# ChampiB/CBO_with_OOP

Measured on NVIDIA B200. Metric: EI grid-points/sec per trial (all exploration sets), higher is better.
Workload: dtype f64

## Files before the change

cbo_with_oop_b200/build.py:

```python
from __future__ import annotations

import os
import subprocess
import sys
from concurrent.futures import ThreadPoolExecutor

HERE = os.path.dirname(os.path.abspath(__file__))
CSRC = os.path.join(HERE, "csrc")
INCLUDE = os.path.join(HERE, "..", "include")
LIB = os.path.join(HERE, "libcbo_b200.so")
SOURCES = ["api.cu", "tables.cu", "prior_precompute.cu", "prior_eval.cu", "prior_pair.cu", "prior_rows.cu", "posterior_fit.cu", "sweep.cu", "obs_gp_fit.cu", "sem.cu", "refine.cu"]
HEADERS = ["cbo_common.cuh", "dmma_tile.cuh", "dmma_tma_tile.cuh", "prior_pair.cuh", os.path.join(INCLUDE, "cbo_b200.h")]
NVCC_FLAGS = ["-gencode", "arch=compute_100a,code=sm_100a", "-O3", "-lineinfo", "-std=c++17",
              "-Xcompiler", "-fPIC", "-Xcompiler", "-fvisibility=hidden"]


def _nvcc() -> str:
    for cand in (os.environ.get("NVCC"), "/usr/local/cuda/bin/nvcc", "nvcc"):
        if cand and (os.path.isabs(cand) and os.path.exists(cand) or not os.path.isabs(cand)):
            return cand
    raise RuntimeError("nvcc not found")


def _stale() -> bool:
    if not os.path.exists(LIB):
        return True
    t = os.path.getmtime(LIB)
    deps = [os.path.join(CSRC, s) for s in SOURCES] + [h if os.path.isabs(h) else os.path.join(CSRC, h) for h in HEADERS]
    deps.append(os.path.abspath(__file__))
    return any(os.path.getmtime(d) > t for d in deps)


def build_library(force: bool = False, verbose: bool = False) -> str:
    if not force and not _stale():
        return LIB
    nvcc = _nvcc()
    objdir = os.path.join(HERE, "build")
    os.makedirs(objdir, exist_ok=True)
    extra = ["-Xptxas", "-v"] if verbose else []
    extra += os.environ.get("CBO_NVCC_EXTRA", "").split()

    def compile_one(src: str) -> str:
        obj = os.path.join(objdir, src.replace(".cu", ".o"))
        cmd = [nvcc, *NVCC_FLAGS, *extra, "-I", INCLUDE, "-c", os.path.join(CSRC, src), "-o", obj]
        r = subprocess.run(cmd, capture_output=True, text=True)
        if r.returncode != 0:
            raise RuntimeError(f"nvcc failed on {src}:\n{r.stdout}\n{r.stderr}")
        if verbose:
            sys.stderr.write(r.stderr)
        return obj

    with ThreadPoolExecutor(max_workers=len(SOURCES)) as ex:
        objs = list(ex.map(compile_one, SOURCES))
    cmd = [nvcc, "-shared", "-o", LIB, *objs, "-gencode", "arch=compute_100a,code=sm_100a"]
    r = subprocess.run(cmd, capture_output=True, text=True)
    if r.returncode != 0:
        raise RuntimeError(f"link failed:\n{r.stdout}\n{r.stderr}")
    return LIB


if __name__ == "__main__":
    print(build_library(force="--force" in sys.argv, verbose="--verbose" in sys.argv))
```

cbo_with_oop_b200/csrc/prior_eval.cu:

```cuda
#include "dmma_tile.cuh"
#include "prior_pair.cuh"

namespace cbo {

constexpr int kPriorWsHeader = 256;

constexpr int kPartialDoubles = 2 * CBO_PRIOR_TILE;
constexpr int kKbPerJ = kMBlkRows / kBK;
constexpr int kPartialFloor = 1024;

struct PriorSplit { int chunk, nsplit, skip_pair; };
__host__ __device__ inline long long prior_tiles(const cbo_set_desc& S, PriorSplit sp) {
    if (!computes_prior(S) || (sp.skip_pair && pair_eligible(S))) return 0;
    return (S.g_count + CBO_PRIOR_TILE - 1) / CBO_PRIOR_TILE;
}
__host__ __device__ inline int prior_nJ(const cbo_set_desc& S) { return (S.n_obs + kMBlkRows - 1) / kMBlkRows; }

__host__ __device__ inline long long prior_G(int n, int chunk) {
    if (n <= 0) return 0;
    const long long q = n / chunk, r = n - q * chunk;
    return (long long)chunk * q * (q + 1) / 2 + r * (q + 1);
}
__host__ __device__ inline long long prior_F(int jb, int chunk) { return prior_G(jb - 1, chunk) + jb; }
__host__ __device__ inline int prior_nsplit(const cbo_set_desc& S, int nsplit) {
    const int nJ = prior_nJ(S), cap = nJ / 2 > 1 ? nJ / 2 : 1;
    return nsplit < cap ? nsplit : cap;
}
__host__ __device__ inline long long prior_items_per_tile(const cbo_set_desc& S, PriorSplit sp) {
    return sp.chunk > 0 ? prior_F(prior_nJ(S), sp.chunk) : prior_nsplit(S, sp.nsplit);
}
__host__ __device__ inline long long prior_items(const cbo_set_desc& S, PriorSplit sp) {
    return prior_tiles(S, sp) * prior_items_per_tile(S, sp);
}

template <int WM_, int WN_, int MA_, int NB_, int STAGES_>
struct PriorCfg {
    static constexpr int WM = WM_, WN = WN_, MA = MA_, NB = NB_, STAGES = STAGES_;
    static constexpr int BM = WM * MA * 8;
    static constexpr int BN = WN * NB * 8;
    static constexpr int NCONS = WM * WN * 32;
    static constexpr int NT = NCONS + 128;
    static constexpr int A_TILE = BM * kBK;
    static constexpr int B_TILE = BN * kBK;
    static constexpr unsigned STAGE_BYTES = (A_TILE + B_TILE) * sizeof(double);
    static constexpr size_t SMEM = (size_t)STAGES * STAGE_BYTES + 2 * WN * BM * sizeof(double) +
                                   (CBO_MAX_D + 1) * BM * sizeof(int32_t) + 2 * STAGES * sizeof(uint64_t) + 16;
    static constexpr int LAUNCH_REGS = (65536 / NT) / 8 * 8;
    static constexpr int PROD_REGS = 40, CONS_REGS = 232;
    static_assert(BM == CBO_PRIOR_TILE, "host item count assumes CBO_PRIOR_TILE points per work item");
    static_assert(BN == kMBlkRows, "the J block must match the row block of M's blocked layout");
    static_assert(NCONS % 128 == 0, "setmaxnreg works on whole warpgroups");
    static_assert(128 * PROD_REGS + NCONS * CONS_REGS <= NT * LAUNCH_REGS, "setmaxnreg budget exceeds the CTA's register pool");
};

struct PriorItem {
    const cbo_set_desc* S;
    int tile, nJ, jb0, jb1, kt0, kt1, sp, ns;
    int kmax;
    bool split;
    bool partial;
    __device__ __forceinline__ bool mine(int jb) const { const int r = jb % (2 * ns); return r == sp || r == 2 * ns - 1 - sp; }
    template <bool SPLIT> __device__ __forceinline__ int kbeg(int jb) const { return SPLIT ? kt0 : 0; }
    template <bool SPLIT> __device__ __forceinline__ int kend(int jb) const {
        const int e = SPLIT ? kt1 : (jb + 1) * kKbPerJ;
        return e < kmax ? e : kmax;
    }
};

constexpr int kMaxBases = 32;
struct PriorBases { int n; int base[kMaxBases + 1]; };

__device__ __forceinline__ PriorItem decode_prior_item(const cbo_set_desc* __restrict__ sets, int num_sets, PriorSplit split,
                                                       const PriorBases& pb, int item) {
    const int chunk = split.chunk;
    int local = item, s = 0;
    if (pb.n == num_sets) {
#pragma unroll 1
        for (; s < num_sets - 1; ++s)
            if (item < pb.base[s + 1]) break;
        local = item - pb.base[s];
    } else {
        for (; s < num_sets - 1; ++s) {
            const int cnt = (int)prior_items(sets[s], split);
            if (local < cnt) break;
            local -= cnt;
        }
    }
    PriorItem it;
    it.S = sets + s;
    it.nJ = prior_nJ(sets[s]);
    it.kmax = (sets[s].n_obs + kBK - 1) / kBK;
    it.split = chunk > 0;
    it.sp = 0, it.ns = 1;
    if (!it.split) {
        it.ns = prior_nsplit(sets[s], split.nsplit);
        it.tile = local / it.ns, it.sp = local % it.ns;
        it.jb0 = 0, it.jb1 = it.nJ, it.kt0 = it.kt1 = 0;
        it.partial = it.ns > 1;
        return it;
    }
    it.partial = prior_F(it.nJ, chunk) > 1;
    const int per_tile = (int)prior_F(it.nJ, chunk);
    it.tile = local / per_tile;
    const int seg = local - it.tile * per_tile;
    int lo = 0, hi = it.nJ - 1;
    while (lo < hi) {
        const int mid = (lo + hi + 1) >> 1;
        if (prior_F(mid, chunk) <= seg) lo = mid; else hi = mid - 1;
    }
    const int jb = lo, piece = seg - (int)prior_F(jb, chunk), lower = (jb + chunk - 1) / chunk;
    it.jb0 = jb, it.jb1 = jb + 1;
    if (piece < lower) {
        const int b1 = (piece + 1) * chunk < jb ? (piece + 1) * chunk : jb;
        it.kt0 = piece * chunk * kKbPerJ, it.kt1 = b1 * kKbPerJ;
    } else {
        it.kt0 = jb * kKbPerJ, it.kt1 = (jb + 1) * kKbPerJ;
    }
    return it;
}

__device__ __forceinline__ void bar_all(int nthreads) { asm volatile("bar.sync 0, %0;" ::"r"(nthreads) : "memory"); }
__device__ __forceinline__ void bar_consumers(int nthreads) { asm volatile("bar.sync 1, %0;" ::"r"(nthreads) : "memory"); }

template <class Cfg, int MW, int NW, int MA2, int NB2>
__device__ __forceinline__ void consume_ragged_block(const PriorItem& it, const double* __restrict__ sA, const double* __restrict__ sB,
                                                     double* __restrict__ sRed, uint64_t* full, uint64_t* empty, int& stage,
                                                     unsigned& phase, const double* __restrict__ scratch, const double* __restrict__ w,
                                                     int warp, int lane) {
    constexpr int BM = Cfg::BM, BN = Cfg::BN, WN = Cfg::WN, STAGES = Cfg::STAGES;
    static_assert(MW * NW * 32 == Cfg::NCONS && MW * MA2 * 8 == BM && NW <= WN, "re-tiling must cover the 128 rows with all consumer warps");
    const int jb = it.nJ - 1, noff = jb * kKbPerJ, ke = it.kmax;
    const int row0 = (warp / NW) * MA2 * 8, wn2 = warp % NW, col0 = wn2 * NB2 * 8;
    double acc[MA2][NB2][2];
#pragma unroll
    for (int mi = 0; mi < MA2; ++mi)
#pragma unroll
        for (int ni = 0; ni < NB2; ++ni) acc[mi][ni][0] = acc[mi][ni][1] = 0.0;
    auto run = [&](int k0, int k1) {
#pragma unroll 1
        for (int kt = k0; kt < k1; ++kt) {
            mbar_wait(&full[stage], phase);
            mma_stage<BM, BN, MA2, NB2, MA2>(sA + stage * Cfg::A_TILE, sB + stage * Cfg::B_TILE, acc, row0, col0, lane);
            __syncwarp();
            if (lane == 0) mbar_arrive(&empty[stage]);
            if (++stage == STAGES) { stage = 0; phase ^= 1u; }
        }
    };
    run(0, noff);
#pragma unroll
    for (int mi = 0; mi < MA2; ++mi)
#pragma unroll
        for (int ni = 0; ni < NB2; ++ni) { acc[mi][ni][0] *= 2.0; acc[mi][ni][1] *= 2.0; }
    run(noff, ke);
    bar_consumers(Cfg::NCONS);
#pragma unroll
    for (int mi = 0; mi < MA2; ++mi) {
        const int r = row0 + mi * 8 + (lane >> 2);
        double q = 0.0, mm = 0.0;
#pragma unroll
        for (int ni = 0; ni < NB2; ++ni) {
            const int j = jb * BN + col0 + ni * 8 + (lane & 3) * 2;
            const double2 u = __ldcg(reinterpret_cast<const double2*>(scratch + (size_t)(j >> 4) * Cfg::A_TILE + frag_off(BM, (j & 15) >> 2, r, j & 3)));
            const double2 ww = ldg_nc_d2(w + j);
            q = fma(acc[mi][ni][0], u.x, q);
            q = fma(acc[mi][ni][1], u.y, q);
            mm = fma(u.x, ww.x, mm);
            mm = fma(u.y, ww.y, mm);
        }
        q += __shfl_xor_sync(0xffffffffu, q, 1);
        q += __shfl_xor_sync(0xffffffffu, q, 2);
        mm += __shfl_xor_sync(0xffffffffu, mm, 1);
        mm += __shfl_xor_sync(0xffffffffu, mm, 2);
        if ((lane & 3) == 0) {
            sRed[wn2 * BM + r] += q;
            sRed[(WN + wn2) * BM + r] += mm;
        }
    }
}

template <class Cfg, int LIVE, bool SPLIT>
__device__ __forceinline__ void consume_item(const PriorItem& it, const double* __restrict__ sA, const double* __restrict__ sB,
                                             double* __restrict__ sRed, uint64_t* full, uint64_t* empty, int& stage, unsigned& phase,
                                             const double* __restrict__ scratch, const double* __restrict__ w, int warp, int lane,
                                             int ragged_cols) {
    constexpr int BM = Cfg::BM, BN = Cfg::BN, MA = Cfg::MA, NB = Cfg::NB, WN = Cfg::WN, STAGES = Cfg::STAGES;
    static_assert(BN / kBK == kKbPerJ, "J block width");
    const int wm = warp / WN, wn = warp % WN;
    const int row0 = wm * MA * 8, col0 = wn * NB * 8;
    if constexpr (LIVE == 0) {
#pragma unroll 1
        for (int jb = it.jb0; jb < it.jb1; ++jb) {
            if (!it.mine(jb)) continue;
#pragma unroll 1
            for (int kt = it.template kbeg<SPLIT>(jb); kt < it.template kend<SPLIT>(jb); ++kt) {
                mbar_wait(&full[stage], phase);
                __syncwarp();
                if (lane == 0) mbar_arrive(&empty[stage]);
                if (++stage == STAGES) { stage = 0; phase ^= 1u; }
            }
        }
        return;
    }
    constexpr int LV = LIVE > 0 ? LIVE : 1;
    double acc[MA][NB][2];
#pragma unroll
    for (int mi = 0; mi < MA; ++mi)
#pragma unroll
        for (int ni = 0; ni < NB; ++ni) acc[mi][ni][0] = acc[mi][ni][1] = 0.0;

    const int jend = (!SPLIT && LIVE == MA && ragged_cols > 0) ? it.nJ - 1 : it.jb1;
#pragma unroll 1
    for (int jb = it.jb0; jb < jend; ++jb) {
        if (!it.mine(jb)) continue;
        const int kb = it.template kbeg<SPLIT>(jb), ke = it.template kend<SPLIT>(jb), noff = jb * kKbPerJ;
        auto double_acc = [&]() {
#pragma unroll
            for (int mi = 0; mi < LV; ++mi)
#pragma unroll
                for (int ni = 0; ni < NB; ++ni) { acc[mi][ni][0] *= 2.0; acc[mi][ni][1] *= 2.0; }
        };
        auto run = [&](int k0, int k1) {
#pragma unroll 1
            for (int kt = k0; kt < k1; ++kt) {
                mbar_wait(&full[stage], phase);
                mma_stage<BM, BN, MA, NB, LV>(sA + stage * Cfg::A_TILE, sB + stage * Cfg::B_TILE, acc, row0, col0, lane);
                __syncwarp();
                if (lane == 0) mbar_arrive(&empty[stage]);
                if (++stage == STAGES) { stage = 0; phase ^= 1u; }
            }
        };
        if constexpr (SPLIT) {
            run(kb, ke);
        } else {
            run(kb, noff);
            double_acc();
            run(noff, ke);
        }
        if (ke <= noff) double_acc();
        const bool with_m = ke > noff;
        const int ubase = !SPLIT ? 0 : (ke <= noff ? noff - (ke - kb) : kb);
#pragma unroll
        for (int mi = 0; mi < LV; ++mi) {
            const int r = row0 + mi * 8 + (lane >> 2);
            double q = 0.0, mm = 0.0;
#pragma unroll
            for (int ni = 0; ni < NB; ++ni) {
                const int j = jb * BN + col0 + ni * 8 + (lane & 3) * 2;
                const double2 u = __ldcg(reinterpret_cast<const double2*>(
                    scratch + (size_t)((j >> 4) - ubase) * Cfg::A_TILE + frag_off(BM, (j & 15) >> 2, r, j & 3)));
                const double2 ww = ldg_nc_d2(w + j);
                q = fma(acc[mi][ni][0], u.x, q);
                q = fma(acc[mi][ni][1], u.y, q);
                mm = fma(u.x, ww.x, mm);
                mm = fma(u.y, ww.y, mm);
                acc[mi][ni][0] = acc[mi][ni][1] = 0.0;
            }
            q += __shfl_xor_sync(0xffffffffu, q, 1);
            q += __shfl_xor_sync(0xffffffffu, q, 2);
            mm += __shfl_xor_sync(0xffffffffu, mm, 1);
            mm += __shfl_xor_sync(0xffffffffu, mm, 2);
            if ((lane & 3) == 0) {
                sRed[wn * BM + r] += q;
                if (with_m) sRed[(WN + wn) * BM + r] += mm;
            }
        }
    }
    if constexpr (!SPLIT && LIVE == MA) {
        if (ragged_cols > 32) consume_ragged_block<Cfg, 4, 2, 4, 4>(it, sA, sB, sRed, full, empty, stage, phase, scratch, w, warp, lane);
        else if (ragged_cols > 16) consume_ragged_block<Cfg, 8, 1, 2, 4>(it, sA, sB, sRed, full, empty, stage, phase, scratch, w, warp, lane);
        else if (ragged_cols > 0) consume_ragged_block<Cfg, 8, 1, 2, 2>(it, sA, sB, sRed, full, empty, stage, phase, scratch, w, warp, lane);
    }
}

template <class Cfg, bool SPLIT>
__global__ void __launch_bounds__(Cfg::NT, 1)
prior_eval_kernel(const cbo_set_desc* __restrict__ sets, int num_sets, PriorSplit split, const PriorBases pb, int total_items,
                  int* __restrict__ counter, double* __restrict__ partials, double* __restrict__ scratch_base, size_t slot_doubles) {
    constexpr int BM = Cfg::BM, BN = Cfg::BN, WN = Cfg::WN, NT = Cfg::NT, NCONS = Cfg::NCONS;
    constexpr int STAGES = Cfg::STAGES;
    extern __shared__ __align__(16) unsigned char smem_raw[];
    double* sA = reinterpret_cast<double*>(smem_raw);
    double* sB = sA + STAGES * Cfg::A_TILE;
    double* sRed = sB + STAGES * Cfg::B_TILE;
    uint64_t* bars = reinterpret_cast<uint64_t*>(sRed + 2 * WN * BM);
    int32_t* sRow = reinterpret_cast<int32_t*>(bars + 2 * STAGES);
    volatile int32_t* sItem = sRow + (CBO_MAX_D + 1) * BM;
    uint64_t* full = bars;
    uint64_t* empty = bars + STAGES;

    const int tid = threadIdx.x, lane = tid & 31, warp = tid >> 5;
    double* __restrict__ scratch = scratch_base + (size_t)blockIdx.x * slot_doubles;

    if (tid == 0) {
        for (int i = 0; i < STAGES; ++i) {
            mbar_init(&full[i], 1);
            mbar_init(&empty[i], Cfg::WM * WN);
        }
        mbar_fence_init();
        *sItem = atomicAdd(counter, 1);
    }
    __syncthreads();
    int stage = 0;
    unsigned phase = 0;

    if (warp >= NCONS / 32) {
        setmaxnreg_dec<Cfg::PROD_REGS>();
        for (;;) {
            const int item = *sItem;
            if (item >= total_items) break;
            const PriorItem it = decode_prior_item(sets, num_sets, split, pb, item);
            const double* __restrict__ M = it.S->M;
            const int Npad = it.S->n_obs_pad;
            bar_all(NT);
            if (warp == NCONS / 32 && lane == 0) {
#pragma unroll 1
                for (int jb = it.jb0; jb < it.jb1; ++jb) {
                    if (!it.mine(jb)) continue;
                    const int kb = it.template kbeg<SPLIT>(jb), ke = it.template kend<SPLIT>(jb);
#pragma unroll 1
                    for (int kt = kb; kt < ke; ++kt) {
                        mbar_wait(&empty[stage], phase ^ 1u);
                        mbar_arrive_expect_tx(&full[stage], Cfg::STAGE_BYTES);
                        bulk_g2s(sB + stage * Cfg::B_TILE, M + mblk_base(jb, kt, Npad), Cfg::B_TILE * sizeof(double), &full[stage]);
                        bulk_g2s(sA + stage * Cfg::A_TILE, scratch + (size_t)(kt - kb) * Cfg::A_TILE, Cfg::A_TILE * sizeof(double), &full[stage]);
                        if (++stage == STAGES) { stage = 0; phase ^= 1u; }
                    }
                }
            }
            __syncwarp();
            bar_all(NT);
        }
    } else {
        setmaxnreg_inc<Cfg::CONS_REGS>();
        for (;;) {
            const int item = *sItem;
            if (item >= total_items) break;
            const PriorItem it = decode_prior_item(sets, num_sets, split, pb, item);
            const cbo_set_desc& S = *it.S;
            const int d = S.points ? 1 : S.d;
            const long long gbeg = S.g_begin, gcnt = S.g_count;
            const int Npad = S.n_obs_pad;
            const int nk_item = SPLIT ? it.kt1 - it.kt0 : it.nJ * kKbPerJ;
            const bool extra = SPLIT && it.kt1 <= it.jb0 * kKbPerJ;
            const int nKT = nk_item + (extra ? kKbPerJ : 0);
            const long long left = gcnt - (long long)it.tile * BM;
            const int nlive = left < BM ? (int)left : BM;

            const bool small_grid = S.g_total < 0x7fffffffLL;
            for (int r = tid; r < BM; r += NCONS) {
                const bool live = r < nlive;
                const long long g0 = gbeg + (live ? (long long)it.tile * BM + r : 0);
                if (small_grid) {
                    unsigned gg = (unsigned)g0;
#pragma unroll
                    for (int k = CBO_MAX_D - 1; k >= 0; --k) {
                        if (k < d) {
                            const unsigned pk = S.points ? (unsigned)S.g_total : (unsigned)S.p[k], q = gg / pk;
                            sRow[k * BM + r] = (int)(gg - q * pk) * Npad;
                            gg = q;
                        }
                    }
                } else {
                    long long gg = g0;
#pragma unroll
                    for (int k = CBO_MAX_D - 1; k >= 0; --k) {
                        if (k < d) {
                            const long long pk = S.points ? S.g_total : (long long)S.p[k];
                            sRow[k * BM + r] = (int)(gg % pk) * Npad;
                            gg /= pk;
                        }
                    }
                }
                sRow[CBO_MAX_D * BM + r] = live ? 1 : 0;
            }
            for (int i = tid; i < 2 * WN * BM; i += NCONS) sRed[i] = 0.0;
            bar_consumers(NCONS);

            {
                const double* tab[CBO_MAX_D];
#pragma unroll
                for (int k = 0; k < CBO_MAX_D; ++k) tab[k] = S.tab[k < d ? k : 0];
                const int per_slab = ((nlive + 3) >> 2) * 32;
                constexpr int UW = (BM / 4 * 32 + NCONS - 1) / NCONS;
                int roff[UW][CBO_MAX_D], dst0[UW], j0[UW];
                bool valid[UW], live[UW];
#pragma unroll
                for (int x = 0; x < UW; ++x) {
                    const int wi = tid + x * NCONS, l = wi & 31;
                    const int kb = l >> 3, half = l & 1, row = (wi >> 5) * 4 + ((l & 7) >> 1);
                    valid[x] = wi < per_slab;
                    live[x] = valid[x] && sRow[CBO_MAX_D * BM + row] != 0;
                    j0[x] = kb * 4 + half * 2;
                    dst0[x] = frag_off(BM, kb, row, half * 2);
#pragma unroll
                    for (int k = 0; k < CBO_MAX_D; ++k) roff[x][k] = (k < d && valid[x]) ? sRow[k * BM + row] : 0;
                }
#pragma unroll 1
                for (int ks = 0; ks < nKT; ++ks) {
                    const int kt = !SPLIT ? ks : (ks < nk_item ? it.kt0 + ks : it.jb0 * kKbPerJ + (ks - nk_item));
                    double2 v[UW];
#pragma unroll
                    for (int x = 0; x < UW; ++x) {
                        v[x] = make_double2(0.0, 0.0);
                        if (live[x]) {
                            const int j = kt * kBK + j0[x];
                            v[x] = ldg_nc_d2(tab[0] + roff[x][0] + j);
#pragma unroll
                            for (int k = 1; k < CBO_MAX_D; ++k) {
                                if (k < d) {
                                    const double2 t = ldg_nc_d2(tab[k] + roff[x][k] + j);
                                    v[x].x *= t.x; v[x].y *= t.y;
                                }
                            }
                        }
                    }
#pragma unroll
                    for (int x = 0; x < UW; ++x)
                        if (valid[x]) *reinterpret_cast<double2*>(scratch + (size_t)ks * Cfg::A_TILE + dst0[x]) = v[x];
                }
                fence_proxy_async();
            }
            bar_all(NT);

            {
                const int live_here = nlive - (warp / WN) * Cfg::MA * 8;
                const int need = live_here <= 0 ? 0 : (live_here + 7) >> 3;
                const int lc = S.n_obs - (it.nJ - 1) * BN;
                const int ragged_cols = (!SPLIT && nlive == BM && it.nJ > 1 && lc <= 64 && it.mine(it.nJ - 1)) ? lc : 0;
#define CBO_CONSUME(LIVE) consume_item<Cfg, LIVE, SPLIT>(it, sA, sB, sRed, full, empty, stage, phase, scratch, S.w, warp, lane, ragged_cols)
                if (need >= 7) CBO_CONSUME(8);
                else if (need == 6) CBO_CONSUME(6);
                else if (need == 5) CBO_CONSUME(5);
                else if (need == 4) CBO_CONSUME(4);
                else if (need == 3) CBO_CONSUME(3);
                else if (need == 2) CBO_CONSUME(2);
                else if (need == 1) CBO_CONSUME(1);
                else CBO_CONSUME(0);
#undef CBO_CONSUME
            }
            bar_consumers(NCONS);

            double* out_m = S.m;
            double* out_v = S.v;
            for (int r = tid; r < nlive; r += NCONS) {
                const long long loc = (long long)it.tile * BM + r;
                double qs = 0.0, ms = 0.0;
#pragma unroll
                for (int x = 0; x < WN; ++x) { qs += sRed[x * BM + r]; ms += sRed[(WN + x) * BM + r]; }
                if (it.partial) {
                    partials[(size_t)item * kPartialDoubles + r] = qs;
                    partials[(size_t)item * kPartialDoubles + BM + r] = ms;
                } else {
                    out_m[loc] = ms;
                    out_v[loc] = (S.s2 + S.noise) - qs;
                }
            }
            bar_consumers(NCONS);
            if (tid == 0) *sItem = atomicAdd(counter, 1);
            bar_all(NT);
        }
    }
}

__global__ void __launch_bounds__(CBO_PRIOR_TILE)
prior_finalize_kernel(const cbo_set_desc* __restrict__ sets, int num_sets, PriorSplit split,
                      const double* __restrict__ partials) {
    long long base = 0;
    for (int s = 0; s < num_sets; ++s) {
        const cbo_set_desc& S = sets[s];
        const int tiles = (int)prior_tiles(S, split);
        if (tiles == 0) continue;
        const int per = (int)prior_items_per_tile(S, split);
        if (per > 1) {
            const long long gcnt = S.g_count;
            double* out_m = S.m;
            double* out_v = S.v;
            for (int tile = blockIdx.x; tile < tiles; tile += gridDim.x) {
                const int r = threadIdx.x;
                const long long loc = (long long)tile * CBO_PRIOR_TILE + r;
                if (loc < gcnt) {
                    double qs = 0.0, ms = 0.0;
                    const double* p = partials + (size_t)(base + (long long)tile * per) * kPartialDoubles;
                    for (int i = 0; i < per; ++i, p += kPartialDoubles) {
                        qs += p[r];
                        ms += p[CBO_PRIOR_TILE + r];
                    }
                    out_m[loc] = ms;
                    out_v[loc] = (S.s2 + S.noise) - qs;
                }
            }
        }
        base += (long long)tiles * per;
    }
}

using PriorCfgA = PriorCfg<2, 4, 8, 4, 4>;

static size_t prior_slot_doubles(const cbo_set_desc* h_sets, int num_sets) {
    int npad = 0;
    for (int s = 0; s < num_sets; ++s)
        if (computes_prior(h_sets[s]) && h_sets[s].n_obs_pad > npad) npad = h_sets[s].n_obs_pad;
    return (size_t)CBO_PRIOR_TILE * npad;
}

static size_t prior_partial_items(long long ctas) { return (size_t)(4 * ctas + kPartialFloor); }

size_t prior_rows_workspace_bytes(const cbo_set_desc* h_sets, int num_sets);
int prior_rows_impl(const cbo_set_desc* h_sets, const cbo_set_desc* d_sets, int num_sets, void* d_ws, size_t ws_bytes,
                    size_t ws_offset, cudaStream_t st);

static size_t pair_area_bytes(const cbo_set_desc* h_sets, int num_sets) {
    return (pair_area_doubles(h_sets, num_sets) * sizeof(double) + 255) / 256 * 256;
}

size_t prior_workspace_bytes_impl(const cbo_set_desc* h_sets, int num_sets, int num_ctas) {
    const size_t grid = pair_area_bytes(h_sets, num_sets) + prior_partial_items(num_ctas) * kPartialDoubles * sizeof(double) +
                        (size_t)num_ctas * prior_slot_doubles(h_sets, num_sets) * sizeof(double);
    const size_t rows = prior_rows_workspace_bytes(h_sets, num_sets);
    return kPriorWsHeader + (grid > rows ? grid : rows);
}

double prior_eval_flops_impl(const cbo_set_desc* h_sets, int num_sets, int num_sms) {
    const bool pair = pair_items_total(h_sets, num_sets) >= num_sms;
    double fl = 0.0;
    for (int s = 0; s < num_sets; ++s) {
        const cbo_set_desc& S = h_sets[s];
        if (!computes_prior(S) || S.g_count == 0) continue;
        if (pair && pair_eligible(S)) {
            const PairGeom g = pair_geom(S);
            double blocks = 0.0;
            for (int ca = 0; ca < g.nchA; ++ca)
                for (int cb = 0; cb < g.nchB; ++cb) {
                    const int ra = g.pa - ca * g.CRa, rb = g.pb - cb * g.CRb;
                    blocks += (double)(((ra < g.CRa ? ra : g.CRa) + 7) / 8) * (((rb < g.CRb ? rb : g.CRb) + 7) / 8);
                }
            fl += 2.0 * 64.0 * blocks * g.s_count * (double)g.Kslabs * kBK;
        } else {
            const int nJ = prior_nJ(S), lc = S.n_obs - (nJ - 1) * kMBlkRows;
            const int last_cols = (nJ == 1 || lc > 64) ? 128 : (lc <= 16 ? 16 : (lc <= 32 ? 32 : 64));
            const double n16 = (double)((S.n_obs + kBK - 1) / kBK * kBK);
            fl += (double)S.g_count * 2.0 * (128.0 * 128.0 * (nJ - 1) * nJ / 2.0 + last_cols * n16);
        }
    }
    return fl;
}

int prior_eval_impl(const cbo_set_desc* h_sets, const cbo_set_desc* d_sets, int num_sets, int which, void* d_ws,
                    size_t ws_bytes, cudaStream_t st) {
    if (which == 1) return prior_rows_impl(h_sets, d_sets, num_sets, d_ws, ws_bytes, kPriorWsHeader, st);
    int dev = 0, sms = 0;
    CBO_CUDA(cudaGetDevice(&dev));
    CBO_CUDA(cudaDeviceGetAttribute(&sms, cudaDevAttrMultiProcessorCount, dev));
    const size_t slot = prior_slot_doubles(h_sets, num_sets);
    const size_t fixed = kPriorWsHeader + (size_t)kPartialFloor * kPartialDoubles * sizeof(double);
    const size_t per_cta = 4 * kPartialDoubles * sizeof(double) + slot * sizeof(double);
    size_t pair_bytes = pair_area_bytes(h_sets, num_sets);
    if (d_ws == nullptr || ws_bytes < fixed + per_cta + pair_bytes) pair_bytes = 0;
    PriorSplit split{0, 1, 0};
    if (pair_bytes > 0 && pair_items_total(h_sets, num_sets) >= sms) split.skip_pair = 1;
    if (split.skip_pair) {
        const int rc = prior_pair_impl(h_sets, d_sets, num_sets, reinterpret_cast<double*>(static_cast<unsigned char*>(d_ws) + kPriorWsHeader),
                                       sms, st);
        if (rc != 0) return rc;
    }
    long long tiles = 0;
    for (int s = 0; s < num_sets; ++s) {
        const cbo_set_desc& S = h_sets[s];
        if (prior_tiles(S, split) == 0) continue;
        for (int k = 0; k < (S.points ? 1 : S.d); ++k) {
            const long long pk = S.points ? S.g_total : (long long)S.p[k];
            CBO_REQUIRE(pk * (long long)S.n_obs_pad < 2147483647LL, "cbo_prior_eval: table %d of set %d too large", k, s);
        }
        CBO_REQUIRE((long long)CBO_PRIOR_TILE * S.n_obs_pad < 2147483647LL, "cbo_prior_eval: set %d n_obs_pad too large", s);
        tiles += prior_tiles(S, split);
    }
    if (tiles == 0) return 0;
    CBO_REQUIRE(d_ws != nullptr && ws_bytes >= fixed + per_cta + pair_bytes,
                "cbo_prior_eval: workspace of %zu bytes cannot hold one scratch slot (%zu bytes needed); see cbo_prior_workspace_bytes",
                ws_bytes, fixed + per_cta + pair_bytes);
    long long ctas = (long long)((ws_bytes - fixed - pair_bytes) / per_cta);
    if (ctas > sms) ctas = sms;
    auto count = [&](PriorSplit sp) {
        long long t = 0;
        for (int s = 0; s < num_sets; ++s) t += prior_items(h_sets[s], sp);
        return t;
    };
    if (tiles < 2 * ctas) {
        int nJmax = 1;
        for (int s = 0; s < num_sets; ++s)
            if (prior_tiles(h_sets[s], split) > 0 && prior_nJ(h_sets[s]) > nJmax) nJmax = prior_nJ(h_sets[s]);
        const long long budget = (long long)prior_partial_items(ctas) < 4 * ctas ? (long long)prior_partial_items(ctas) : 4 * ctas;
        for (int c = 1; c <= nJmax && nJmax > 1; ++c)
            if (count(PriorSplit{c, 1, split.skip_pair}) <= budget) { split.chunk = c; break; }
        if (split.chunk == 0) {
            split.nsplit = (int)((2 * ctas + tiles - 1) / tiles);
            while (split.nsplit > 1 && count(split) > (long long)prior_partial_items(ctas)) --split.nsplit;
        }
    }
    const long long total = count(split);
    const bool partial = split.chunk > 0 || split.nsplit > 1;
    CBO_REQUIRE(total < 2147483647LL, "cbo_prior_eval: too many work items");
    CBO_REQUIRE(!partial || (size_t)total <= prior_partial_items(ctas), "cbo_prior_eval: internal: partial buffer too small");
    const long long grid = ctas < total ? ctas : total;
    unsigned char* ws = reinterpret_cast<unsigned char*>(d_ws);
    double* partials = reinterpret_cast<double*>(ws + kPriorWsHeader + pair_bytes);
    double* scratch = partials + prior_partial_items(ctas) * kPartialDoubles;
    auto kern = split.chunk > 0 ? prior_eval_kernel<PriorCfgA, true> : prior_eval_kernel<PriorCfgA, false>;
    CBO_CUDA(allow_dynamic_smem(prior_eval_kernel<PriorCfgA, true>, PriorCfgA::SMEM));
    CBO_CUDA(allow_dynamic_smem(prior_eval_kernel<PriorCfgA, false>, PriorCfgA::SMEM));
    CBO_CUDA(cudaMemsetAsync(d_ws, 0, kPriorWsHeader, st));
    PriorBases pb;
    pb.n = num_sets <= kMaxBases ? num_sets : 0;
    pb.base[0] = 0;
    for (int s = 0; s < kMaxBases; ++s)
        pb.base[s + 1] = pb.base[s] + (s < pb.n ? (int)prior_items(h_sets[s], split) : 0);
    kern<<<(unsigned)grid, PriorCfgA::NT, PriorCfgA::SMEM, st>>>(d_sets, num_sets, split, pb, (int)total,
                                                                 reinterpret_cast<int*>(ws), partials, scratch, slot);
    note_launch();
    CBO_CUDA(cudaGetLastError());
    if (partial) {
        prior_finalize_kernel<<<(unsigned)(tiles < 1024 ? tiles : 1024), CBO_PRIOR_TILE, 0, st>>>(d_sets, num_sets, split, partials);
        note_launch();
        CBO_CUDA(cudaGetLastError());
    }
    return 0;
}

}
```

Baseline: 341,400.

## Emulate f64 prior quadratic form with int8 tcgen05 MMA via CRT moduli

Adds an int8 tensor-core path for the prior variance quadratic form. It scales f64 rows and the M matrix to integers, splits them into 16 small-modulus residues, runs tcgen05 kind::i8 MMAs per modulus, and rebuilds exact values with CRT before compensated f64 accumulation. It targets sets with large n_obs and many tiles, where the DMMA f64 path is compute-bound. The trade-off is heavy residue conversion and CRT work, plus a large per-CTA scratch workspace, and the path only triggers when that workspace fits.

After: 447,600 (median of 6 runs). +31.1%, better.

```diff
diff --git a/cbo_with_oop_b200/build.py b/cbo_with_oop_b200/build.py
--- a/cbo_with_oop_b200/build.py
+++ b/cbo_with_oop_b200/build.py
@@ -9,7 +9,7 @@
 CSRC = os.path.join(HERE, "csrc")
 INCLUDE = os.path.join(HERE, "..", "include")
 LIB = os.path.join(HERE, "libcbo_b200.so")
-SOURCES = ["api.cu", "tables.cu", "prior_precompute.cu", "prior_eval.cu", "prior_pair.cu", "prior_rows.cu", "posterior_fit.cu", "sweep.cu", "obs_gp_fit.cu", "sem.cu", "refine.cu"]
+SOURCES = ["api.cu", "tables.cu", "prior_precompute.cu", "prior_eval.cu", "prior_i8.cu", "prior_pair.cu", "prior_rows.cu", "posterior_fit.cu", "sweep.cu", "obs_gp_fit.cu", "sem.cu", "refine.cu"]
 HEADERS = ["cbo_common.cuh", "dmma_tile.cuh", "dmma_tma_tile.cuh", "prior_pair.cuh", os.path.join(INCLUDE, "cbo_b200.h")]
 NVCC_FLAGS = ["-gencode", "arch=compute_100a,code=sm_100a", "-O3", "-lineinfo", "-std=c++17",
               "-Xcompiler", "-fPIC", "-Xcompiler", "-fvisibility=hidden"]
diff --git a/cbo_with_oop_b200/csrc/prior_eval.cu b/cbo_with_oop_b200/csrc/prior_eval.cu
--- a/cbo_with_oop_b200/csrc/prior_eval.cu
+++ b/cbo_with_oop_b200/csrc/prior_eval.cu
@@ -1,5 +1,5 @@
 #include "dmma_tile.cuh"
-#include "prior_pair.cuh"
+#include "prior_i8.cuh"
 
 namespace cbo {
 
@@ -9,9 +9,9 @@
 constexpr int kKbPerJ = kMBlkRows / kBK;
 constexpr int kPartialFloor = 1024;
 
-struct PriorSplit { int chunk, nsplit, skip_pair; };
+struct PriorSplit { int chunk, nsplit, skip_pair, i8_min_tiles; };
 __host__ __device__ inline long long prior_tiles(const cbo_set_desc& S, PriorSplit sp) {
-    if (!computes_prior(S) || (sp.skip_pair && pair_eligible(S))) return 0;
+    if (!computes_prior(S) || (sp.skip_pair && pair_eligible(S)) || i8_eligible(S, sp.i8_min_tiles, sp.skip_pair)) return 0;
     return (S.g_count + CBO_PRIOR_TILE - 1) / CBO_PRIOR_TILE;
 }
 __host__ __device__ inline int prior_nJ(const cbo_set_desc& S) { return (S.n_obs + kMBlkRows - 1) / kMBlkRows; }
@@ -517,7 +517,14 @@
     const size_t grid = pair_area_bytes(h_sets, num_sets) + prior_partial_items(num_ctas) * kPartialDoubles * sizeof(double) +
                         (size_t)num_ctas * prior_slot_doubles(h_sets, num_sets) * sizeof(double);
     const size_t rows = prior_rows_workspace_bytes(h_sets, num_sets);
-    return kPriorWsHeader + (grid > rows ? grid : rows);
+    size_t i8 = 0;
+    for (int s = 0; s < num_sets; ++s)
+        if (i8_eligible(h_sets[s], 1, true)) {
+            const size_t b = prior_i8_workspace_bytes(h_sets[s], num_ctas);
+            if (b > i8) i8 = b;
+        }
+    const size_t big = grid > rows ? grid : rows;
+    return kPriorWsHeader + (big > i8 ? big : i8);
 }
 
 double prior_eval_flops_impl(const cbo_set_desc* h_sets, int num_sets, int num_sms) {
@@ -556,12 +563,28 @@
     const size_t per_cta = 4 * kPartialDoubles * sizeof(double) + slot * sizeof(double);
     size_t pair_bytes = pair_area_bytes(h_sets, num_sets);
     if (d_ws == nullptr || ws_bytes < fixed + per_cta + pair_bytes) pair_bytes = 0;
-    PriorSplit split{0, 1, 0};
+    PriorSplit split{0, 1, 0, 0};
     if (pair_bytes > 0 && pair_items_total(h_sets, num_sets) >= sms) split.skip_pair = 1;
     if (split.skip_pair) {
         const int rc = prior_pair_impl(h_sets, d_sets, num_sets, reinterpret_cast<double*>(static_cast<unsigned char*>(d_ws) + kPriorWsHeader),
                                        sms, st);
         if (rc != 0) return rc;
+    }
+    {
+        size_t need = 0;
+        for (int s = 0; s < num_sets; ++s)
+            if (i8_eligible(h_sets[s], 2 * sms, split.skip_pair)) {
+                const size_t b = prior_i8_workspace_bytes(h_sets[s], sms);
+                if (b > need) need = b;
+            }
+        if (need > 0 && d_ws != nullptr && ws_bytes >= kPriorWsHeader + need) {
+            split.i8_min_tiles = 2 * sms;
+            for (int s = 0; s < num_sets; ++s)
+                if (i8_eligible(h_sets[s], split.i8_min_tiles, split.skip_pair)) {
+                    const int rc = prior_i8_impl(h_sets[s], d_sets + s, static_cast<unsigned char*>(d_ws) + kPriorWsHeader, sms, st);
+                    if (rc != 0) return rc;
+                }
+        }
     }
     long long tiles = 0;
     for (int s = 0; s < num_sets; ++s) {
@@ -591,7 +614,7 @@
             if (prior_tiles(h_sets[s], split) > 0 && prior_nJ(h_sets[s]) > nJmax) nJmax = prior_nJ(h_sets[s]);
         const long long budget = (long long)prior_partial_items(ctas) < 4 * ctas ? (long long)prior_partial_items(ctas) : 4 * ctas;
         for (int c = 1; c <= nJmax && nJmax > 1; ++c)
-            if (count(PriorSplit{c, 1, split.skip_pair}) <= budget) { split.chunk = c; break; }
+            if (count(PriorSplit{c, 1, split.skip_pair, split.i8_min_tiles}) <= budget) { split.chunk = c; break; }
         if (split.chunk == 0) {
             split.nsplit = (int)((2 * ctas + tiles - 1) / tiles);
             while (split.nsplit > 1 && count(split) > (long long)prior_partial_items(ctas)) --split.nsplit;
diff --git a/cbo_with_oop_b200/csrc/prior_i8.cu b/cbo_with_oop_b200/csrc/prior_i8.cu
--- /dev/null
+++ b/cbo_with_oop_b200/csrc/prior_i8.cu
@@ -0,0 +1,410 @@
+#include "dmma_tile.cuh"
+#include "prior_i8.cuh"
+
+#include <cmath>
+
+namespace cbo {
+
+constexpr int kI8Mods = 16, kI8Stages = 4, kI8StageK = 128, kI8Threads = 192;
+constexpr unsigned kI8ABytes = 128 * kI8StageK, kI8BBytes = kI8Chunk * kI8StageK, kI8StageBytes = kI8ABytes + kI8BBytes;
+
+__constant__ int c_mod[kI8Mods] = {256, 255, 253, 251, 247, 241, 239, 233, 229, 227, 223, 217, 211, 199, 197, 193};
+__constant__ double c_inv_mod[kI8Mods] = {1.0 / 256, 1.0 / 255, 1.0 / 253, 1.0 / 251, 1.0 / 247, 1.0 / 241, 1.0 / 239, 1.0 / 233,
+                                          1.0 / 229, 1.0 / 227, 1.0 / 223, 1.0 / 217, 1.0 / 211, 1.0 / 199, 1.0 / 197, 1.0 / 193};
+__constant__ unsigned c_w[kI8Mods][4] = {
+    {0x02e00f01u, 0x38869293u, 0xc414656fu, 0x055a110au}, {0x1e9b2000u, 0xa14a062au, 0xfb6e9b40u, 0x247850d7u},
+    {0x1789df00u, 0xb05acfa5u, 0xe2f2d2c3u, 0x1fffd89au}, {0xbbbd6700u, 0x87f9916bu, 0xacf04661u, 0x19f80a3fu},
+    {0x100dd100u, 0xb97d6303u, 0x2b052a8bu, 0x16b10abbu}, {0x0d14b500u, 0xc1cc75f8u, 0x648a1736u, 0x00dc8191u},
+    {0x2799c800u, 0x4a076123u, 0x9b984ac8u, 0x1ff687bbu}, {0x7d646f00u, 0xc9cfaa52u, 0x134a76b4u, 0x29292a13u},
+    {0x151d0600u, 0xc340b57bu, 0x505de66cu, 0x05705dbeu}, {0x0d603f00u, 0xadc43fa0u, 0x2e79c7ffu, 0x16dca3fau},
+    {0x74905e00u, 0xdb0d2a75u, 0x43831857u, 0x0654790au}, {0xbb44ad00u, 0x490b99d0u, 0x89424a89u, 0x0d33892au},
+    {0xb8ff4e00u, 0xf617dc87u, 0x9aee4461u, 0x1b2745cfu}, {0xb14f0b00u, 0xb41649fbu, 0x86dd427cu, 0x096367ecu},
+    {0xd63c3900u, 0x0bcd579bu, 0xe8e217d6u, 0x1a57e7d4u}, {0x03d6f400u, 0x62cc34aeu, 0xf2435d63u, 0x18f40d0eu}};
+__constant__ unsigned c_p[4] = {0xa9b2e100u, 0x49e5694du, 0xbaccc54fu, 0x2984652cu};
+constexpr double kInvP = 1.8120609044457363e-38;
+static const int kModuliHost[kI8Mods] = {256, 255, 253, 251, 247, 241, 239, 233, 229, 227, 223, 217, 211, 199, 197, 193};
+
+__host__ __device__ inline size_t i8_b_mod_bytes(int nJ) { return (size_t)nJ * (nJ + 1) * kI8BBytes; }
+__host__ __device__ inline size_t i8_cta_bytes(int kpad) {
+    return (size_t)kI8Mods * 128 * kpad
+           + (size_t)128 * kpad * sizeof(double)
+           + (size_t)kI8Mods * 128 * kI8Chunk;
+}
+
+__device__ __forceinline__ int sym_residue(double V, int l) {
+    const double p = (double)c_mod[l];
+    int r = (int)fma(-p, rint(V * c_inv_mod[l]), V);
+    const int hi = (c_mod[l] - 1) >> 1, lo = -(c_mod[l] >> 1);
+    if (r > hi) r -= c_mod[l];
+    if (r < lo) r += c_mod[l];
+    return r;
+}
+__device__ __forceinline__ int scale_exp(double amax, int bits) {
+    if (!(amax > 0.0)) return 0;
+    int E;
+    frexp(amax, &E);
+    return bits - E;
+}
+__device__ __forceinline__ unsigned box_off(int rows, int n, int k) {
+    return (unsigned)((k >> 5) * rows * 32 + (n >> 3) * 256 + ((k >> 4) & 1) * 128 + (n & 7) * 16 + (k & 15));
+}
+
+__global__ void i8_mscale_kernel(const cbo_set_desc* __restrict__ d_set, int* __restrict__ sexp, int kpad, int mbits) {
+    const cbo_set_desc& S = *d_set;
+    const int j = blockIdx.x * blockDim.x + threadIdx.x;
+    if (j >= kpad) return;
+    double amax = 0.0;
+    if (j < S.n_obs_pad) {
+        const int jb = j / kMBlkRows, kend = (jb + 1) * kMBlkRows;
+        for (int k = 0; k < kend; ++k) {
+            const double c = (k / kMBlkRows < jb) ? 2.0 : 1.0;
+            amax = fmax(amax, fabs(c * S.M[mblk_off(j, k, S.n_obs_pad)]));
+        }
+    }
+    sexp[j] = scale_exp(amax, mbits);
+}
+
+__global__ void i8_mres_kernel(const cbo_set_desc* __restrict__ d_set, const int* __restrict__ sexp, int8_t* __restrict__ B, int nJ) {
+    const cbo_set_desc& S = *d_set;
+    const int j = blockIdx.x * blockDim.x + threadIdx.x, k0 = blockIdx.y * 16;
+    const int J = j / kI8Chunk, n = j % kI8Chunk;
+    if (J >= nJ || k0 >= kI8Chunk * (J + 1)) return;
+    const int npad = S.n_obs_pad, jb = j / kMBlkRows, e = sexp[j];
+    double V[16];
+#pragma unroll
+    for (int i = 0; i < 16; ++i) {
+        const int k = k0 + i, kb = k / kMBlkRows;
+        double m = 0.0;
+        if (j < npad && k < npad && kb <= jb) m = (kb < jb ? 2.0 : 1.0) * S.M[mblk_off(j, k, npad)];
+        V[i] = rint(ldexp(m, e));
+    }
+    const size_t off = (size_t)J * (J + 1) * kI8BBytes + (size_t)(k0 / kI8StageK) * kI8BBytes + box_off(kI8Chunk, n, k0 % kI8StageK);
+    const size_t bmod = i8_b_mod_bytes(nJ);
+    for (int l = 0; l < kI8Mods; ++l) {
+        unsigned w[4];
+#pragma unroll
+        for (int q = 0; q < 4; ++q) {
+            unsigned x = 0;
+#pragma unroll
+            for (int b = 0; b < 4; ++b) x |= (unsigned)(sym_residue(V[4 * q + b], l) & 0xff) << (8 * b);
+            w[q] = x;
+        }
+        *reinterpret_cast<uint4*>(B + l * bmod + off) = make_uint4(w[0], w[1], w[2], w[3]);
+    }
+}
+
+__device__ __forceinline__ uint64_t umma_desc(unsigned addr) {
+    return (uint64_t)((addr & 0x3FFFF) >> 4) | ((uint64_t)(128 >> 4) << 16) | ((uint64_t)(256 >> 4) << 32) | (1ull << 46);
+}
+__device__ __forceinline__ void i8_wait(uint64_t* bar, unsigned parity) {
+    unsigned ok = 0;
+    while (!ok)
+        asm volatile("{\n\t.reg .pred p;\n\tmbarrier.try_wait.parity.shared::cta.b64 p, [%1], %2;\n\tselp.u32 %0, 1, 0, p;\n\t}"
+                     : "=r"(ok) : "r"(smem_u32(bar)), "r"(parity) : "memory");
+}
+__device__ __forceinline__ void umma_commit(uint64_t* bar) {
+    asm volatile("tcgen05.commit.cta_group::1.mbarrier::arrive::one.shared::cluster.b64 [%0];" ::"r"(smem_u32(bar)) : "memory");
+}
+
+__device__ __forceinline__ void limb_norm(long long d[4]) {
+#pragma unroll
+    for (int i = 0; i < 3; ++i) {
+        const long long c = d[i] >> 32;
+        d[i] -= c * 4294967296LL;
+        d[i + 1] += c;
+    }
+}
+
+__device__ __forceinline__ double crt_value(const unsigned r[kI8Mods]) {
+    unsigned long long s[4] = {0, 0, 0, 0};
+#pragma unroll
+    for (int l = 0; l < kI8Mods; ++l)
+#pragma unroll
+        for (int i = 0; i < 4; ++i) s[i] += (unsigned long long)r[l] * c_w[l][i];
+    const double approx = (((double)s[3] * 4294967296.0 + (double)s[2]) * 4294967296.0 + (double)s[1]) * 4294967296.0 + (double)s[0];
+    const long long q = (long long)rint(approx * kInvP);
+    long long d[4];
+#pragma unroll
+    for (int i = 0; i < 4; ++i) d[i] = (long long)s[i] - q * (long long)c_p[i];
+    limb_norm(d);
+    const bool neg = d[3] < 0;
+    if (neg) {
+#pragma unroll
+        for (int i = 0; i < 4; ++i) d[i] = -d[i];
+        limb_norm(d);
+    }
+    const unsigned long long top = ((unsigned long long)d[3] << 32) | (unsigned long long)d[2];
+    const unsigned long long low = ((unsigned long long)d[1] << 32) | (unsigned long long)d[0];
+    const double t = fma((double)top, 18446744073709551616.0, (double)low);
+    return neg ? -t : t;
+}
+
+__global__ void __launch_bounds__(kI8Threads, 1)
+prior_i8_kernel(const cbo_set_desc* __restrict__ d_set, const int8_t* __restrict__ B, const int* __restrict__ sexp,
+                unsigned char* __restrict__ scratch_base, int tiles, int nJ) {
+    extern __shared__ __align__(1024) uint8_t smem[];
+    __shared__ __align__(8) uint64_t full[kI8Stages], empty[kI8Stages], accfull[2], accempty[2];
+    __shared__ uint32_t tmem_base;
+    __shared__ int sRow[CBO_MAX_D][128];
+    __shared__ unsigned long long sMax[128];
+    __shared__ int sExp[128];
+    const cbo_set_desc& S = *d_set;
+    const int tid = threadIdx.x, warp = tid >> 5, lane = tid & 31;
+    const int npad = S.n_obs_pad, kpad = nJ * kI8Chunk, d = S.d;
+    const int kslabs = (S.n_obs + kI8StageK - 1) / kI8StageK;
+    unsigned char* scr = scratch_base + (size_t)blockIdx.x * i8_cta_bytes(kpad);
+    int8_t* Ares = reinterpret_cast<int8_t*>(scr);
+    double* Ud = reinterpret_cast<double*>(scr + (size_t)kI8Mods * 128 * kpad);
+    uint8_t* Rres = scr + (size_t)kI8Mods * 128 * kpad + (size_t)128 * kpad * sizeof(double);
+    const size_t a_mod = (size_t)128 * kpad, b_mod = i8_b_mod_bytes(nJ);
+
+    if (warp == 0) {
+        asm volatile("tcgen05.alloc.cta_group::1.sync.aligned.shared::cta.b32 [%0], %1;" ::"r"(smem_u32(&tmem_base)), "r"(512u) : "memory");
+        asm volatile("tcgen05.relinquish_alloc_permit.cta_group::1.sync.aligned;" ::: "memory");
+    }
+    if (tid == 32) {
+        for (int s = 0; s < kI8Stages; ++s) { mbar_init(&full[s], 1); mbar_init(&empty[s], 1); }
+        for (int b = 0; b < 2; ++b) { mbar_init(&accfull[b], 1); mbar_init(&accempty[b], 128); }
+        mbar_fence_init();
+    }
+    asm volatile("tcgen05.fence::before_thread_sync;" ::: "memory");
+    __syncthreads();
+    asm volatile("tcgen05.fence::after_thread_sync;" ::: "memory");
+    const uint32_t tm = tmem_base;
+    unsigned it = 0, acc_it = 0;
+
+    for (int tile = blockIdx.x; tile < tiles; tile += gridDim.x) {
+        const long long left = S.g_count - (long long)tile * 128;
+        const int nlive = left < 128 ? (int)left : 128;
+        for (int r = tid; r < 128; r += kI8Threads) {
+            long long gg = S.g_begin + (long long)tile * 128 + (r < nlive ? r : 0);
+            for (int k = CBO_MAX_D - 1; k >= 0; --k)
+                if (k < d) {
+                    const long long pk = S.p[k];
+                    sRow[k][r] = (int)(gg % pk) * npad;
+                    gg /= pk;
+                }
+            sMax[r] = 0ull;
+        }
+        __syncthreads();
+        const int units = 128 * (kpad / 16);
+        for (int u = tid; u < units; u += kI8Threads) {
+            const int r = u % 128, k0 = (u / 128) * 16;
+            double v[16];
+#pragma unroll
+            for (int i = 0; i < 16; ++i) v[i] = 0.0;
+            if (r < nlive && k0 < npad) {
+#pragma unroll
+                for (int i = 0; i < 16; i += 2) {
+                    double2 x = ldg_nc_d2(S.tab[0] + sRow[0][r] + k0 + i);
+                    for (int k = 1; k < d; ++k) {
+                        const double2 t = ldg_nc_d2(S.tab[k] + sRow[k][r] + k0 + i);
+                        x.x *= t.x; x.y *= t.y;
+                    }
+                    v[i] = x.x; v[i + 1] = x.y;
+                }
+            }
+            double amax = 0.0;
+#pragma unroll
+            for (int i = 0; i < 16; i += 2) {
+                *reinterpret_cast<double2*>(Ud + (size_t)r * kpad + k0 + i) = make_double2(v[i], v[i + 1]);
+                amax = fmax(amax, fmax(fabs(v[i]), fabs(v[i + 1])));
+            }
+            atomicMax(&sMax[r], (unsigned long long)__double_as_longlong(amax));
+        }
+        __syncthreads();
+        for (int r = tid; r < 128; r += kI8Threads) sExp[r] = scale_exp(__longlong_as_double((long long)sMax[r]), 53);
+        __syncthreads();
+        for (int u = tid; u < units; u += kI8Threads) {
+            const int r = u % 128, k0 = (u / 128) * 16, e = sExp[r];
+            double V[16];
+#pragma unroll
+            for (int i = 0; i < 16; i += 2) {
+                const double2 x = *reinterpret_cast<const double2*>(Ud + (size_t)r * kpad + k0 + i);
+                V[i] = rint(ldexp(x.x, e)); V[i + 1] = rint(ldexp(x.y, e));
+            }
+            const size_t off = (size_t)(k0 / kI8StageK) * kI8ABytes + box_off(128, r, k0 % kI8StageK);
+            for (int l = 0; l < kI8Mods; ++l) {
+                unsigned w[4];
+#pragma unroll
+                for (int q = 0; q < 4; ++q) {
+                    unsigned x = 0;
+#pragma unroll
+                    for (int b = 0; b < 4; ++b) x |= (unsigned)(sym_residue(V[4 * q + b], l) & 0xff) << (8 * b);
+                    w[q] = x;
+                }
+                *reinterpret_cast<uint4*>(Ares + l * a_mod + off) = make_uint4(w[0], w[1], w[2], w[3]);
+            }
+        }
+        fence_proxy_async();
+        asm volatile("tcgen05.fence::before_thread_sync;" ::: "memory");
+        __syncthreads();
+        asm volatile("tcgen05.fence::after_thread_sync;" ::: "memory");
+
+        if (warp == 0) {
+            if (lane == 0) {
+                for (int J = 0; J < nJ; ++J) {
+                    const int ns = 2 * (J + 1) < kslabs ? 2 * (J + 1) : kslabs;
+                    for (int l = 0; l < kI8Mods; ++l) {
+                        const int8_t* a = Ares + l * a_mod;
+                        const int8_t* b = B + l * b_mod + (size_t)J * (J + 1) * kI8BBytes;
+                        for (int s = 0; s < ns; ++s, ++it) {
+                            const unsigned st = it % kI8Stages, ph = (it / kI8Stages) & 1u;
+                            i8_wait(&empty[st], ph ^ 1u);
+                            uint8_t* dst = smem + st * kI8StageBytes;
+                            mbar_arrive_expect_tx(&full[st], kI8StageBytes);
+                            bulk_g2s(dst, a + (size_t)s * kI8ABytes, kI8ABytes, &full[st]);
+                            bulk_g2s(dst + kI8ABytes, b + (size_t)s * kI8BBytes, kI8BBytes, &full[st]);
+                        }
+                    }
+                }
+            } else {
+                for (int J = 0; J < nJ; ++J) it += kI8Mods * (2 * (J + 1) < kslabs ? 2 * (J + 1) : kslabs);
+            }
+            acc_it += nJ * kI8Mods;
+        } else if (warp == 1) {
+            const uint32_t idesc = (2u << 4) | (1u << 7) | (1u << 10) | ((256u >> 3) << 17) | ((128u >> 4) << 24);
+            for (int J = 0; J < nJ; ++J) {
+                const int ns = 2 * (J + 1) < kslabs ? 2 * (J + 1) : kslabs;
+                for (int l = 0; l < kI8Mods; ++l, ++acc_it) {
+                    if (lane == 0) {
+                        const unsigned buf = acc_it & 1u, aph = (acc_it >> 1) & 1u;
+                        i8_wait(&accempty[buf], aph ^ 1u);
+                        asm volatile("tcgen05.fence::after_thread_sync;" ::: "memory");
+                        const uint32_t dt = tm + buf * 256u;
+                        for (int s = 0; s < ns; ++s) {
+                            const unsigned st = (it + s) % kI8Stages, ph = ((it + s) / kI8Stages) & 1u;
+                            i8_wait(&full[st], ph);
+                            asm volatile("tcgen05.fence::after_thread_sync;" ::: "memory");
+                            const unsigned sa = smem_u32(smem + st * kI8StageBytes), sb = sa + kI8ABytes;
+#pragma unroll
+                            for (int k = 0; k < kI8StageK / 32; ++k) {
+                                const uint64_t da = umma_desc(sa + k * 4096), db = umma_desc(sb + k * 8192);
+                                const uint32_t accumulate = (s > 0 || k > 0);
+                                asm volatile("{\n\t.reg .pred p;\n\tsetp.ne.b32 p, %4, 0;\n\t"
+                                             "tcgen05.mma.cta_group::1.kind::i8 [%0], %1, %2, %3, p;\n\t}"
+                                             ::"r"(dt), "l"(da), "l"(db), "r"(idesc), "r"(accumulate) : "memory");
+                            }
+                            umma_commit(&empty[st]);
+                        }
+                        umma_commit(&accfull[buf]);
+                    }
+                    it += ns;
+                }
+            }
+        } else {
+            const int r = 32 * (warp & 3) + lane;
+            const uint32_t lane_base = (uint32_t)(32 * (warp & 3)) << 16;
+            const int e_x = sExp[r];
+            const double* __restrict__ urow = Ud + (size_t)r * kpad;
+            double qs = 0.0, qc = 0.0, ms = 0.0;
+            for (int J = 0; J < nJ; ++J) {
+                for (int l = 0; l < kI8Mods; ++l, ++acc_it) {
+                    const unsigned buf = acc_it & 1u, aph = (acc_it >> 1) & 1u;
+                    i8_wait(&accfull[buf], aph);
+                    asm volatile("tcgen05.fence::after_thread_sync;" ::: "memory");
+                    const int p = c_mod[l];
+                    const double pd = (double)p, ip = c_inv_mod[l];
+#pragma unroll 1
+                    for (int c = 0; c < kI8Chunk; c += 32) {
+                        uint32_t v[32];
+                        asm volatile(
+                            "tcgen05.ld.sync.aligned.32x32b.x32.b32 {%0,%1,%2,%3,%4,%5,%6,%7,%8,%9,%10,%11,%12,%13,%14,%15,"
+                            "%16,%17,%18,%19,%20,%21,%22,%23,%24,%25,%26,%27,%28,%29,%30,%31}, [%32];"
+                            : "=r"(v[0]), "=r"(v[1]), "=r"(v[2]), "=r"(v[3]), "=r"(v[4]), "=r"(v[5]), "=r"(v[6]), "=r"(v[7]),
+                              "=r"(v[8]), "=r"(v[9]), "=r"(v[10]), "=r"(v[11]), "=r"(v[12]), "=r"(v[13]), "=r"(v[14]), "=r"(v[15]),
+                              "=r"(v[16]), "=r"(v[17]), "=r"(v[18]), "=r"(v[19]), "=r"(v[20]), "=r"(v[21]), "=r"(v[22]), "=r"(v[23]),
+                              "=r"(v[24]), "=r"(v[25]), "=r"(v[26]), "=r"(v[27]), "=r"(v[28]), "=r"(v[29]), "=r"(v[30]), "=r"(v[31])
+                            : "r"(tm + lane_base + buf * 256u + (uint32_t)c) : "memory");
+                        asm volatile("tcgen05.wait::ld.sync.aligned;" ::: "memory");
+                        unsigned w[8];
+#pragma unroll
+                        for (int q = 0; q < 8; ++q) {
+                            unsigned x = 0;
+#pragma unroll
+                            for (int b = 0; b < 4; ++b) {
+                                const double a = (double)(int)v[4 * q + b];
+                                int rr = (int)fma(-pd, rint(a * ip), a);
+                                if (rr < 0) rr += p;
+                                if (rr >= p) rr -= p;
+                                x |= (unsigned)rr << (8 * b);
+                            }
+                            w[q] = x;
+                        }
+                        uint4* dst = reinterpret_cast<uint4*>(Rres + ((size_t)l * 128 + r) * kI8Chunk + c);
+                        dst[0] = make_uint4(w[0], w[1], w[2], w[3]);
+                        dst[1] = make_uint4(w[4], w[5], w[6], w[7]);
+                    }
+                    asm volatile("tcgen05.fence::before_thread_sync;" ::: "memory");
+                    mbar_arrive(&accempty[buf]);
+                }
+                if (r < nlive) {
+#pragma unroll 1
+                    for (int c = 0; c < kI8Chunk; c += 16) {
+                        const int j0 = J * kI8Chunk + c;
+                        if (j0 >= npad) break;
+                        uint4 rv[kI8Mods];
+#pragma unroll
+                        for (int l = 0; l < kI8Mods; ++l) rv[l] = *reinterpret_cast<const uint4*>(Rres + ((size_t)l * 128 + r) * kI8Chunk + c);
+#pragma unroll 1
+                        for (int i = 0; i < 16; ++i) {
+                            unsigned res[kI8Mods];
+#pragma unroll
+                            for (int l = 0; l < kI8Mods; ++l) {
+                                const unsigned word = (i < 4 ? rv[l].x : i < 8 ? rv[l].y : i < 12 ? rv[l].z : rv[l].w);
+                                res[l] = (word >> (8 * (i & 3))) & 0xffu;
+                            }
+                            const int j = j0 + i;
+                            const double t = ldexp(crt_value(res), -(e_x + sexp[j]));
+                            const double uj = urow[j];
+                            const double pr = __dmul_rn(uj, t), pe = fma(uj, t, -pr), sn = __dadd_rn(qs, pr), bb = __dsub_rn(sn, qs);
+                            qc += pe + __dadd_rn(__dsub_rn(qs, __dsub_rn(sn, bb)), __dsub_rn(pr, bb));
+                            qs = sn;
+                            ms = fma(uj, S.w[j], ms);
+                        }
+                    }
+                }
+            }
+            if (r < nlive) {
+                const long long loc = (long long)tile * 128 + r;
+                S.m[loc] = ms;
+                S.v[loc] = (S.s2 + S.noise) - (qs + qc);
+            }
+        }
+        asm volatile("tcgen05.fence::before_thread_sync;" ::: "memory");
+        __syncthreads();
+        asm volatile("tcgen05.fence::after_thread_sync;" ::: "memory");
+    }
+    if (warp == 0) asm volatile("tcgen05.dealloc.cta_group::1.sync.aligned.b32 %0, %1;" ::"r"(tm), "r"(512u) : "memory");
+}
+
+size_t prior_i8_workspace_bytes(const cbo_set_desc& S, int num_ctas) {
+    const int nJ = i8_chunks(S), kpad = nJ * kI8Chunk;
+    return (kI8Mods * i8_b_mod_bytes(nJ) + 255) / 256 * 256 + ((size_t)kpad * sizeof(int) + 255) / 256 * 256 +
+           (size_t)num_ctas * i8_cta_bytes(kpad);
+}
+
+int prior_i8_impl(const cbo_set_desc& h, const cbo_set_desc* d_set, unsigned char* ws, int ctas, cudaStream_t st) {
+    const int nJ = i8_chunks(h), kpad = nJ * kI8Chunk;
+    double log2p = 0.0;
+    for (int l = 0; l < kI8Mods; ++l) log2p += std::log2((double)kModuliHost[l]);
+    const int mbits = (int)std::floor(log2p - 2.0 - 53.0 - std::log2((double)kpad));
+    int8_t* B = reinterpret_cast<int8_t*>(ws);
+    int* sexp = reinterpret_cast<int*>(ws + (kI8Mods * i8_b_mod_bytes(nJ) + 255) / 256 * 256);
+    unsigned char* scratch = reinterpret_cast<unsigned char*>(sexp) + ((size_t)kpad * sizeof(int) + 255) / 256 * 256;
+    i8_mscale_kernel<<<(kpad + 127) / 128, 128, 0, st>>>(d_set, sexp, kpad, mbits);
+    note_launch();
+    CBO_CUDA(cudaGetLastError());
+    i8_mres_kernel<<<dim3((unsigned)(kpad + 127) / 128, (unsigned)(kpad / 16)), 128, 0, st>>>(d_set, sexp, B, nJ);
+    note_launch();
+    CBO_CUDA(cudaGetLastError());
+    const long long tiles = (h.g_count + 127) / 128;
+    const size_t smem = (size_t)kI8Stages * kI8StageBytes;
+    CBO_CUDA(allow_dynamic_smem(prior_i8_kernel, smem));
+    prior_i8_kernel<<<(unsigned)(ctas < tiles ? ctas : tiles), kI8Threads, smem, st>>>(d_set, B, sexp, scratch, (int)tiles, nJ);
+    note_launch();
+    CBO_CUDA(cudaGetLastError());
+    return 0;
+}
+
+}
diff --git a/cbo_with_oop_b200/csrc/prior_i8.cuh b/cbo_with_oop_b200/csrc/prior_i8.cuh
--- /dev/null
+++ b/cbo_with_oop_b200/csrc/prior_i8.cuh
@@ -0,0 +1,20 @@
+#pragma once
+#include "prior_pair.cuh"
+
+namespace cbo {
+
+constexpr int kI8Chunk = 256;
+constexpr int kI8MaxK = 131071 / kI8Chunk * kI8Chunk;
+constexpr int kI8MinNpad = 2048;
+
+__host__ __device__ inline int i8_chunks(const cbo_set_desc& S) { return (S.n_obs + kI8Chunk - 1) / kI8Chunk; }
+
+__host__ __device__ inline bool i8_eligible(const cbo_set_desc& S, int min_tiles, bool skip_pair) {
+    return min_tiles > 0 && computes_prior(S) && !S.points && !(skip_pair && pair_eligible(S)) && S.g_count > 0 &&
+           S.n_obs_pad >= kI8MinNpad && i8_chunks(S) * kI8Chunk <= kI8MaxK && (S.g_count + CBO_PRIOR_TILE - 1) / CBO_PRIOR_TILE >= min_tiles;
+}
+
+size_t prior_i8_workspace_bytes(const cbo_set_desc& S, int num_ctas);
+int prior_i8_impl(const cbo_set_desc& h, const cbo_set_desc* d_set, unsigned char* ws, int ctas, cudaStream_t st);
+
+}
```
